# pkzhou/PointSLOT

Hardware: AMD Instinct MI355X
Metric: tracked frames/sec KITTI stereo 1242x375 (higher is better)
Workload: dtype u8

## Files before the change

include/pointslot_hip.h:

```cpp
#ifndef POINTSLOT_HIP_H
#define POINTSLOT_HIP_H

#include <stddef.h>
#include <stdint.h>

#ifdef __cplusplus
extern "C" {
#endif

typedef enum ps_status {
  PS_OK = 0,
  PS_ERR_INVALID = -1,
  PS_ERR_HIP = -2,
  PS_ERR_CAPACITY = -3,
  PS_ERR_NO_DEVICE = -4
} ps_status;

typedef struct ps_keypoint {
  float x, y;
  float size;
  float angle;
  float response;
  int32_t octave;
  int32_t class_id;
} ps_keypoint;

const char* ps_last_error(void);
int ps_device_count(int* count);
const char* ps_version(void);
int ps_debug_poison_lds(int device, uint32_t pattern);
int ps_debug_mfma_f64_peak(int device, double* tflops);
int ps_debug_traffic_kernel(int device, int mode, size_t bytes, int repeats);
void* ps_pinned_alloc(size_t bytes);
void ps_pinned_free(void* p);

typedef struct ps_orb ps_orb;

typedef struct ps_orb_config {
  int32_t nfeatures;
  float scale_factor;
  int32_t nlevels;
  int32_t ini_th_fast;
  int32_t min_th_fast;
  int32_t max_batch;
  int32_t device;
} ps_orb_config;

int ps_orb_create(const ps_orb_config* cfg, ps_orb** out);
void ps_orb_destroy(ps_orb* h);

int ps_orb_get_tables(const ps_orb* h, float* scale_factors, float* inv_scale_factors,
                      float* level_sigma2, float* inv_level_sigma2, int32_t* features_per_level);

int ps_orb_level_size(const ps_orb* h, int w, int hgt, int level, int32_t* w_l, int32_t* h_l);

int ps_orb_extract(ps_orb* h, const uint8_t* img, int w, int hgt, int stride, ps_keypoint* kps,
                   uint8_t* desc, int cap, int* n, uint8_t* const* pyramid_out);

int ps_orb_extract_masked(ps_orb* h, const uint8_t* img, const uint8_t* mask, int w, int hgt, int stride, int mask_stride,
                          ps_keypoint* kps, uint8_t* desc, int cap, int* n);

typedef struct ps_cvorb ps_cvorb;
int ps_cvorb_create(int nfeatures, float scale_factor, int nlevels, int edge_threshold, int fast_threshold, int device, ps_cvorb** out);
void ps_cvorb_destroy(ps_cvorb* h);
int ps_cvorb_detect_and_compute(ps_cvorb* h, const uint8_t* img, const uint8_t* mask, int w, int hgt, int stride, int mask_stride,
                                ps_keypoint* kps, uint8_t* desc, int cap, int* n);
int ps_cvorb_debug_read(ps_cvorb* h, int level, int what, void* out, size_t out_bytes, int* n);

int ps_cvorb_detect_batch_device(ps_cvorb* h, const uint8_t* d_imgs, const uint8_t* d_masks, int nimg, int w, int hgt, int stride,
                                 size_t image_pitch, int mask_stride, size_t mask_pitch, void* stream);
int ps_cvorb_batch_device_outputs(const ps_cvorb* h, const ps_keypoint** d_kps, const uint8_t** d_desc, const int32_t** d_counts,
                                  const int32_t** d_overflow, int32_t* capacity);
int ps_cvorb_batch_fetch(ps_cvorb* h, int image, ps_keypoint* kps, uint8_t* desc, int cap, int* n);

int ps_orb_extract_batch_device(ps_orb* h, const uint8_t* d_imgs, int nimg, int w, int hgt, int stride,
                                size_t image_pitch, void* stream);
int ps_orb_batch_device_outputs(const ps_orb* h, const ps_keypoint** d_kps, const uint8_t** d_desc,
                                const int32_t** d_counts, int32_t* kp_capacity);
int ps_orb_batch_fetch(ps_orb* h, int image, ps_keypoint* kps, uint8_t* desc, int cap, int* n);
int ps_orb_sync(ps_orb* h);

int ps_orb_extract_batch(ps_orb* h, const uint8_t* const* imgs, int nimg, int w, int hgt, int stride);

int ps_orb_stereo_match_batch(ps_orb* h, int npairs, float mb, float mbf);
int ps_orb_stereo_device_outputs(const ps_orb* h, const float** d_uright, const float** d_depth, const int32_t** d_kept);
int ps_orb_stereo_fetch(ps_orb* h, int pair, float* u_right, float* depth, int cap, int* n_left, int* kept);
int ps_orb_stereo_match_pair(ps_orb* left, ps_orb* right, float mb, float mbf, float* u_right, float* depth, int cap, int* n_left);
typedef struct ps_stereo_frame {
  ps_keypoint* kps; uint8_t* desc; float* u_right; float* depth;
  int32_t cap;
  int32_t n, n_right, kept;
} ps_stereo_frame;
int ps_orb_stereo_fetch_frames(ps_orb* h, ps_stereo_frame* frames, int npairs);
int ps_orb_stereo_match_keys(ps_orb* left, ps_orb* right, const ps_keypoint* kps_l, const uint8_t* desc_l, int n_left,
                             const ps_keypoint* kps_r, const uint8_t* desc_r, int n_right, float mb, float mbf,
                             float* u_right, float* depth, int* kept);

int ps_orb_debug_read(ps_orb* h, int image, int level, int what, void* out, size_t out_bytes, int* n);

int ps_orb_stage_times(ps_orb* h, const char** names, float* ms, int cap, int* n);
int ps_orb_enable_stage_timing(ps_orb* h, int enable);

typedef struct ps_matcher ps_matcher;
int ps_matcher_create(int device, ps_matcher** out);
void ps_matcher_destroy(ps_matcher* m);
int ps_matcher_last_kernel_ms(const ps_matcher* m, float* ms);

int ps_hamming_matrix(ps_matcher* m, const uint8_t* q, int nq, const uint8_t* t, int nt, uint16_t* out);

int ps_distinctive_descriptors(ps_matcher* m, const uint8_t* desc, const int32_t* off, int npoints, int32_t* best);

typedef struct ps_bf_problem {
  const uint8_t* q_desc; const float* q_angle; const uint8_t* q_valid; int32_t nq;
  const uint8_t* t_desc; const float* t_angle; int32_t nt;
  int32_t* query_of_train;
// ... 287 lines not shown
```

pointslot_amd/csrc/cvorb_host.hip:

```cpp
#include <hip/hip_runtime.h>
#include <math.h>
#include <stdlib.h>
#include <string.h>
#include <algorithm>
#include <vector>
#include "../../include/pointslot_hip.h"
#include "cvorb_plan.h"
#include "ps_common.h"

extern "C" {
void psk_cv_level0(const CvLevelDev*, const uint8_t*, int, const uint8_t*, int, hipStream_t);
void psk_cv_resize(const CvLevelDev*, const CvLevelDev*, const int4*, const int4*, hipStream_t);
void psk_cv_detect(const CvLevelDev*, int, int, int, int32_t*, hipStream_t);
void psk_cv_blur(const CvLevelDev*, const int*, hipStream_t);
void psk_cv_describe(const CvPlanDev*, const CvSel*, int, void*, uint8_t*, hipStream_t);
void psk_cvb_run(const CvbPlan*, int, const uint8_t*, int, size_t, const uint8_t*, int, size_t, int, hipStream_t);
}

struct ps_cvorb {
  int nfeatures, nlevels, edge, fast_th, device;
  double scale_factor;
  hipStream_t stream = nullptr;
  int w = 0, h = 0;
  bool planned = false;
// ... 289 lines not shown
int ps_cvorb_debug_read(ps_cvorb* h, int level, int what, void* out, size_t out_bytes, int* n) {
  if (!h || !h->planned || level < 0 || level >= h->nlevels || !out) return ps_set_error(PS_ERR_INVALID, "ps_cvorb_debug_read: bad argument");
  PS_HIP(hipSetDevice(h->device));
  if (h->last_fast) {
    const int rc = single_host_selected(h, h->w, h->last_had_mask, nullptr, nullptr, 0, nullptr);
    if (rc != PS_OK) return rc;
  }
  PS_HIP(hipDeviceSynchronize());
  const CvLevelDev& L = h->plan.lv[level];
  if (what == 4) { if (out_bytes < 8) return ps_set_error(PS_ERR_CAPACITY, "buffer too small"); ((int32_t*)out)[0] = L.w; ((int32_t*)out)[1] = L.h; return PS_OK; }
  if (what == 3) {
    const std::vector<float>& c = h->last_cand[level];
    if (c.size() * 4 > out_bytes) return ps_set_error(PS_ERR_CAPACITY, "buffer too small");
    if (!c.empty()) memcpy(out, c.data(), c.size() * 4);
    if (n) *n = (int)(c.size() / 4);
    return PS_OK;
  }
  if ((size_t)L.w * L.h > out_bytes) return ps_set_error(PS_ERR_CAPACITY, "buffer too small");
  if (what == 0) PS_HIP(hipMemcpy2D(out, L.w, L.pad + (size_t)CV_BORDER * L.stride + CV_BORDER, L.stride, L.w, L.h, hipMemcpyDeviceToHost));
  else if (what == 1) PS_HIP(hipMemcpy2D(out, L.w, L.blur + (size_t)CV_BORDER * L.stride + CV_BORDER, L.stride, L.w, L.h, hipMemcpyDeviceToHost));
  else if (what == 2) { if (h->last_had_mask) PS_HIP(hipMemcpy(out, L.mask, (size_t)L.w * L.h, hipMemcpyDeviceToHost)); else memset(out, 0, (size_t)L.w * L.h); }
  else return ps_set_error(PS_ERR_INVALID, "unknown `what` %d", what);
  return PS_OK;
}

}

namespace {
int build_batch_plan(ps_cvorb* h, int w, int hgt, int cap) {
  if (h->b_buf) { hipFree(h->b_buf); h->b_buf = nullptr; }
  h->bplanned = false;
  CvbPlan& P = h->bplan;
  memset(&P, 0, sizeof(P));
  P.nlevels = h->nlevels; P.edge = h->edge; P.fast_th = h->fast_th; P.w0 = w; P.h0 = hgt;
  P.ocw = (w + 7) / 8; P.och = (hgt + 7) / 8;
  if (P.ocw > 512) return ps_set_error(PS_ERR_INVALID, "the batched object detector supports images up to 4096 pixels wide");
  {
    const int hp = 15;
    int v, v0, vmax = cv_floor(hp * sqrtf(2.f) / 2 + 1), vmin = cv_ceil(hp * sqrtf(2.f) / 2);
    for (v = 0; v <= vmax; ++v) P.umax[v] = cv_round(sqrt((double)hp * hp - v * v));
    for (v = hp, v0 = 0; v >= vmin; --v) { while (P.umax[v0] == P.umax[v0 + 1]) ++v0; P.umax[v] = v0; ++v0; }
    static const int disc[16] = {15, 15, 15, 15, 14, 14, 14, 13, 13, 12, 11, 10, 9, 8, 6, 3};
    for (v = 0; v <= hp; ++v)
      if (P.umax[v] != disc[v]) return ps_set_error(PS_ERR_INVALID, "the intensity-centroid disc differs from the kernels' mask table");
  }
  for (int i = 0; i < 4; i++) P.kq[i] = h->kq[i];
  std::vector<int> quota(h->nlevels, 0);
  {
    const float factor = (float)(1.0 / h->scale_factor);
    float ndesired = h->nfeatures * (1 - factor) / (1 - (float)pow((double)factor, (double)h->nlevels));
    int sum = 0;
    for (int l = 0; l < h->nlevels - 1; l++) { quota[l] = cv_round(ndesired); sum += quota[l]; ndesired *= factor; }
    quota[h->nlevels - 1] = std::max(h->nfeatures - sum, 0);
  }
  std::vector<std::vector<int4>> xt(h->nlevels), yt(h->nlevels);
  size_t img_off = 0;
  auto take_img = [&](size_t bytes) { size_t r = img_off; img_off += al(bytes + 64); return r; };
  for (int l = 0; l < h->nlevels; l++) {
    CvbLevel& L = P.lv[l];
    L.scale = (float)pow(h->scale_factor, (double)l);
    const float inv_scale = 1.0f / L.scale;
    L.w = cv_round(w * inv_scale); L.h = cv_round(hgt * inv_scale);
    if (L.w <= 2 * h->edge || L.h <= 2 * h->edge || L.w <= 2 * 24 || L.h <= 2 * 24)
      return ps_set_error(PS_ERR_INVALID, "image %dx%d: level %d is %dx%d, too small for the detector", w, hgt, l, L.w, L.h);
    L.stride = (int)((L.w + 2 * CV_BORDER + 63) / 64 * 64);
    L.tw = (L.w + 2 * CV_BORDER + CVB_TILE - 1) / CVB_TILE; L.th = (L.h + 2 * CV_BORDER + CVB_TILE - 1) / CVB_TILE;
    if (L.tw * L.th > CVB_MAX_TILES) return ps_set_error(PS_ERR_INVALID, "the batched object detector supports levels of up to %d tiles", CVB_MAX_TILES);
    L.cw = (L.w + 2 * CV_BORDER + 7) / 8; L.ch = (L.h + 2 * CV_BORDER + 7) / 8;
    L.cw = std::max(L.cw, 4 * L.tw); L.ch = std::max(L.ch, 4 * L.th);
    L.cw = (L.cw + 3) & ~3;
    if (L.cw > 1024 || L.ch > 512) return ps_set_error(PS_ERR_INVALID, "image too large for the batched object detector's planning kernel");
    L.cell_off = P.cell_total; P.cell_total += L.cw * L.ch; P.cell_max = std::max(P.cell_max, L.cw * L.ch);
    L.tile_off = P.tile_total; P.tile_total += L.tw * L.th;
    L.quota = quota[l];
    L.o_pad = take_img((size_t)L.stride * (L.h + 2 * CV_BORDER)); L.o_blur = take_img((size_t)L.stride * (L.h + 2 * CV_BORDER));
    L.o_mask = take_img((size_t)L.w * L.h); L.o_score = 0;
    if (l > 0) {
      exact_table(P.lv[l - 1].w, L.w, xt[l], &L.sx, &L.dminx, &L.dmaxx); exact_table(P.lv[l - 1].h, L.h, yt[l], &L.sy, &L.dminy, &L.dmaxy);
      if ((double)P.lv[l - 1].w / L.w * 32 + 6 > 48 || (double)P.lv[l - 1].h / L.h * 32 + 6 > 48)
        return ps_set_error(PS_ERR_INVALID, "the batched object detector supports scale factors up to 1.3");
    }
  }
  P.arena_pitch = img_off;
  P.ocap = 2048;
  int max_tiles = 0;
  for (int l = 0; l < h->nlevels; l++) max_tiles = std::max(max_tiles, P.lv[l].tw * P.lv[l].th);
  P.wl_cap = cap * max_tiles;
  if (2 * (size_t)P.cell_total + 2 * (size_t)P.cell_max + 2 * (size_t)(P.ocw + 1) * (P.och + 1) + P.tile_total + 64 > 150 * 1024 || P.tile_total > 8 * 512) return ps_set_error(PS_ERR_INVALID, "image too large for the batched object detector's planning kernel");
  size_t off = 0;
  auto take = [&](size_t bytes) { size_t r = off; off += al(bytes + 64); return r; };
  const size_t o_arena = take(P.arena_pitch * (size_t)cap);
  std::vector<size_t> o_xt(h->nlevels, 0), o_yt(h->nlevels, 0);
  for (int l = 1; l < h->nlevels; l++) { o_xt[l] = take(xt[l].size() * 16); o_yt[l] = take(yt[l].size() * 16); }
  const size_t o_wl = take((size_t)3 * CV_MAX_LEVELS * P.wl_cap * 4);
  const size_t o_kpmap = take((size_t)cap * P.cell_total);
  const size_t o_cand = take((size_t)cap * h->nlevels * CVB_CAND_CAP * sizeof(float4));
  const size_t o_sel = take((size_t)cap * h->nlevels * CVB_CAND_CAP * sizeof(CvSel));
  const size_t o_kps = take((size_t)cap * P.ocap * sizeof(ps_keypoint)), o_desc = take((size_t)cap * P.ocap * 32);
  const size_t o_dump = take(1024);
  const size_t z0 = off;
  const size_t o_occ = take((size_t)cap * P.ocw * P.och), o_wlc = take(3 * CV_MAX_LEVELS * 4), o_ncand = take((size_t)cap * h->nlevels * 4);
  const size_t o_nsel = take((size_t)cap * h->nlevels * 4), o_count = take((size_t)cap * 4), o_ovf = take((size_t)cap * 4);
  const size_t z1 = off;
  hipError_t e = hipMalloc(&h->b_buf, off);
  if (e != hipSuccess) return ps_set_error(PS_ERR_HIP, "hipMalloc(%zu): %s", off, hipGetErrorString(e));
  uint8_t* D = h->b_buf;
  if (const char* fill = getenv("PS_DEBUG_FILL")) PS_HIP(hipMemsetAsync(D, atoi(fill), off, h->stream));
  P.arena = D + o_arena;
  for (int l = 1; l < h->nlevels; l++) {
    P.lv[l].xtab = (const int4*)(D + o_xt[l]); P.lv[l].ytab = (const int4*)(D + o_yt[l]);
    PS_HIP(hipMemcpyAsync(D + o_xt[l], xt[l].data(), xt[l].size() * 16, hipMemcpyHostToDevice, h->stream));
    PS_HIP(hipMemcpyAsync(D + o_yt[l], yt[l].data(), yt[l].size() * 16, hipMemcpyHostToDevice, h->stream));
  }
  P.wl = (uint32_t*)(D + o_wl); P.cand = (float4*)(D + o_cand); P.sel = (CvSel*)(D + o_sel);
  P.kps = (ps_keypoint_pod*)(D + o_kps); P.desc = D + o_desc; P.dump = D + o_dump;
  P.occ = D + o_occ; P.kpmap = D + o_kpmap; P.wl_count = (int32_t*)(D + o_wlc); P.ncand = (int32_t*)(D + o_ncand); P.nsel = (int32_t*)(D + o_nsel);
  P.count = (int32_t*)(D + o_count); P.overflow = (int32_t*)(D + o_ovf);
  h->b_zero = D + z0; h->b_zero_bytes = z1 - z0;
  PS_HIP(hipStreamSynchronize(h->stream));
  h->bw = w; h->bh = hgt; h->bcap = cap; h->bplanned = true;
  return PS_OK;
}
}

extern "C" {
hipStream_t psi_cvorb_stream(ps_cvorb* h) { return h->stream; }

int psi_cvorb_batch_begin(ps_cvorb* h, int nimg, int w, int hgt, hipStream_t st, uint8_t** occ, int* ocw, int* och) {
  if (!h->bplanned || h->bw != w || h->bh != hgt || h->bcap < nimg) {
    int rc = build_batch_plan(h, w, hgt, nimg);
    if (rc != PS_OK) return rc;
  }
  PS_HIP(hipMemsetAsync(h->b_zero, 0, h->b_zero_bytes, st));
  if (occ) *occ = h->bplan.occ;
  if (ocw) *ocw = h->bplan.ocw;
  if (och) *och = h->bplan.och;
  return PS_OK;
}
int psi_cvorb_batch_run(ps_cvorb* h, const uint8_t* d_imgs, const uint8_t* d_masks, int nimg, int stride, size_t image_pitch, int mask_stride,
                        size_t mask_pitch, int occupancy_given, hipStream_t st) {
  psk_cvb_run(&h->bplan, nimg, d_imgs, stride, image_pitch, d_masks, mask_stride, mask_pitch, occupancy_given, st);
  PS_HIP(hipGetLastError());
  h->b_last_n = nimg;
  return PS_OK;
}

int psi_cvorb_batch_worklist_counts(ps_cvorb* h, int32_t* counts , int32_t* tiles ) {
  if (!h || !h->bplanned || !counts || !tiles) return ps_set_error(PS_ERR_INVALID, "no batch plan yet");
  PS_HIP(hipSetDevice(h->device));
  PS_HIP(hipDeviceSynchronize());
  PS_HIP(hipMemcpy(counts, h->bplan.wl_count, 3 * CV_MAX_LEVELS * 4, hipMemcpyDeviceToHost));
  for (int l = 0; l < CV_MAX_LEVELS; l++) tiles[l] = l < h->nlevels ? h->bplan.lv[l].tw * h->bplan.lv[l].th : 0;
  return PS_OK;
}

int ps_cvorb_detect_batch_device(ps_cvorb* h, const uint8_t* d_imgs, const uint8_t* d_masks, int nimg, int w, int hgt, int stride, size_t image_pitch,
                                 int mask_stride, size_t mask_pitch, void* stream) {
  if (!h || !d_imgs || !d_masks || nimg < 1 || w < 1 || hgt < 1 || stride < w || mask_stride < w)
    return ps_set_error(PS_ERR_INVALID, "ps_cvorb_detect_batch_device: bad argument");
  PS_HIP(hipSetDevice(h->device));
  hipStream_t st = stream ? (hipStream_t)stream : h->stream;
  int rc = psi_cvorb_batch_begin(h, nimg, w, hgt, st, nullptr, nullptr, nullptr);
  if (rc != PS_OK) return rc;
  return psi_cvorb_batch_run(h, d_imgs, d_masks, nimg, stride, image_pitch, mask_stride, mask_pitch, 0, st);
}

int ps_cvorb_batch_device_outputs(const ps_cvorb* h, const ps_keypoint** d_kps, const uint8_t** d_desc, const int32_t** d_counts,
                                  const int32_t** d_overflow, int32_t* capacity) {
  if (!h || !h->bplanned) return ps_set_error(PS_ERR_INVALID, "no batch plan yet");
  if (d_kps) *d_kps = (const ps_keypoint*)h->bplan.kps;
  if (d_desc) *d_desc = h->bplan.desc;
  if (d_counts) *d_counts = h->bplan.count;
  if (d_overflow) *d_overflow = h->bplan.overflow;
  if (capacity) *capacity = h->bplan.ocap;
  return PS_OK;
}

int ps_cvorb_batch_fetch(ps_cvorb* h, int image, ps_keypoint* kps, uint8_t* desc, int cap, int* n) {
  if (!h || !h->bplanned || image < 0 || image >= h->b_last_n || !n) return ps_set_error(PS_ERR_INVALID, "ps_cvorb_batch_fetch: bad argument");
  PS_HIP(hipSetDevice(h->device));
  PS_HIP(hipDeviceSynchronize());
  int32_t cnt = 0, ovf = 0;
  PS_HIP(hipMemcpy(&cnt, h->bplan.count + image, 4, hipMemcpyDeviceToHost));
  PS_HIP(hipMemcpy(&ovf, h->bplan.overflow + image, 4, hipMemcpyDeviceToHost));
  if (ovf) return ps_set_error(PS_ERR_CAPACITY, "image %d: more than %d FAST keypoints under the mask on a level, or more than %d keypoints in all", image, CVB_CAND_CAP, h->bplan.ocap);
  *n = cnt;
  if (cnt > cap) return ps_set_error(PS_ERR_CAPACITY, "%d keypoints, caller capacity %d", cnt, cap);
  if (cnt > 0) {
    if (!kps || !desc) return ps_set_error(PS_ERR_INVALID, "null output buffer");
    PS_HIP(hipMemcpy(kps, (const ps_keypoint*)h->bplan.kps + (size_t)image * h->bplan.ocap, (size_t)cnt * sizeof(ps_keypoint), hipMemcpyDeviceToHost));
    PS_HIP(hipMemcpy(desc, h->bplan.desc + (size_t)image * h->bplan.ocap * 32, (size_t)cnt * 32, hipMemcpyDeviceToHost));
  }
  return PS_OK;
}
}
```

pointslot_amd/csrc/cvorb_kernels.hip:

```cpp
#include <hip/hip_runtime.h>
#include <stdint.h>
#include <stdlib.h>
#include "cvorb_plan.h"
#include "retain_best.h"

namespace {

#include "describe_common.h"

__constant__ __attribute__((aligned(16))) int8_t cv_pattern[1024] = {
#include "orb_pattern.inc"
};

__device__ __forceinline__ int reflect101(int p, int len) {
  if (len == 1) return 0;
  while (p < 0 || p >= len) p = p < 0 ? -p : 2 * (len - 1) - p;
  return p;
}

__global__ __launch_bounds__(256) void cv_level0(CvLevelDev L, const uint8_t* img, int stride, const uint8_t* mask, int mask_stride) {
  const int px = blockIdx.x * 256 + threadIdx.x, py = blockIdx.y;
  const int PW = L.w + 2 * CV_BORDER;
  if (px >= PW) return;
  const int x = reflect101(px - CV_BORDER, L.w), y = reflect101(py - CV_BORDER, L.h);
  L.pad[(size_t)py * L.stride + px] = img[(size_t)y * stride + x];
  const int ix = px - CV_BORDER, iy = py - CV_BORDER;
  if (L.mask && ix >= 0 && ix < L.w && iy >= 0 && iy < L.h) L.mask[(size_t)iy * L.w + ix] = mask[(size_t)iy * mask_stride + ix];
}

__device__ __forceinline__ uint32_t cv_hline(const uint8_t* S, int sw, int4 tx) {
  if (tx.w == 1) return (uint32_t)S[0] << 8;
  if (tx.w == 2) return (uint32_t)S[sw - 1] << 8;
  return (uint32_t)tx.y * S[tx.x] + (uint32_t)tx.z * S[tx.x + 1];
}
__device__ __forceinline__ uint8_t cv_interp(const uint8_t* src, int sstride, int sw, int sh, int4 tx, int4 ty) {
  if (ty.w != 0) {
    const uint32_t v = cv_hline(src + (size_t)(ty.w == 1 ? 0 : sh - 1) * sstride, sw, tx);
    return (uint8_t)min((v + 128u) >> 8, 255u);
  }
  const uint32_t r0 = cv_hline(src + (size_t)ty.x * sstride, sw, tx), r1 = cv_hline(src + (size_t)(ty.x + 1) * sstride, sw, tx);
  const unsigned long long v = (unsigned long long)r0 * (uint32_t)ty.y + (unsigned long long)r1 * (uint32_t)ty.z;
  return (uint8_t)min((v + 32768ull) >> 16, 255ull);
}
__global__ __launch_bounds__(256) void cv_resize(CvLevelDev L, CvLevelDev P, const int4* xtab, const int4* ytab) {
  const int px = blockIdx.x * 256 + threadIdx.x, py = blockIdx.y;
  const int PW = L.w + 2 * CV_BORDER;
  if (px >= PW) return;
  const int x = reflect101(px - CV_BORDER, L.w), y = reflect101(py - CV_BORDER, L.h);
  const int4 tx = xtab[x], ty = ytab[y];
  const uint8_t* proi = P.pad + (size_t)CV_BORDER * P.stride + CV_BORDER;
  L.pad[(size_t)py * L.stride + px] = cv_interp(proi, P.stride, P.w, P.h, tx, ty);
  const int ix = px - CV_BORDER, iy = py - CV_BORDER;
  if (L.mask && ix >= 0 && ix < L.w && iy >= 0 && iy < L.h) {
    const uint8_t m = cv_interp(P.mask, P.w, P.w, P.h, tx, ty);
    L.mask[(size_t)iy * L.w + ix] = m > 254 ? m : 0;
  }
}

__global__ __launch_bounds__(256) void cv_score(CvLevelDev L, int th) {
  const int x = blockIdx.x * 256 + threadIdx.x, y = blockIdx.y;
  if (x >= L.w) return;
  uint8_t out = 0;
  if (x >= 3 && x < L.w - 3 && y >= 3 && y < L.h - 3) {
    const uint8_t* c = L.pad + (size_t)(CV_BORDER + y) * L.stride + CV_BORDER + x;
    const int st = L.stride, v = c[0];
    const int n = c[3 * st], e = c[3], so = c[-3 * st], w = c[-3];
    const int M = min(min(max(n, e), max(e, so)), min(max(so, w), max(w, n)));
    const int m = max(max(min(n, e), min(e, so)), max(min(so, w), min(w, n)));
    if (v - M > th || m - v > th) {
      const int off[16] = {3 * st, 3 * st + 1, 2 * st + 2, st + 3, 3, -st + 3, -2 * st + 2, -3 * st + 1,
                           -3 * st, -3 * st - 1, -2 * st - 2, -st - 3, -3, st - 3, 2 * st - 2, 3 * st - 1};
      int r[16];
#pragma unroll
      for (int i = 0; i < 16; i++) r[i] = c[off[i]];
      int best = 0;
#pragma unroll
      for (int k = 0; k < 16; k++) {
        int mx = r[k], mn = r[k];
#pragma unroll
        for (int j = 1; j < 9; j++) { mx = max(mx, r[(k + j) & 15]); mn = min(mn, r[(k + j) & 15]); }
        best = max(best, max(v - mx, mn - v));
      }
      if (best > th) out = (uint8_t)best;
    }
  }
  L.score[(size_t)y * L.w + x] = out;
}
// ... 103 lines not shown
__global__ __launch_bounds__(64) void cv_describe(CvPlanDev plan, const CvSel* sel, int nsel, ps_keypoint_pod* kps, uint8_t* desc) {
  const int k = blockIdx.x, lane = threadIdx.x;
  if (k >= nsel) return;
  const CvSel S = sel[k];
  const CvLevelDev& L = plan.lv[S.level];
  const int x0 = S.x, y0 = S.y;
  const uint8_t* center = L.pad + (size_t)(CV_BORDER + y0) * L.stride + CV_BORDER + x0;
  int m10 = 0, m01 = 0;
  if (lane <= 15) {
    const int v = lane, d = plan.umax[v];
    if (v == 0) {
      for (int u = -15; u <= 15; ++u) m10 += u * center[u];
    } else {
      int v_sum = 0;
      for (int u = -d; u <= d; ++u) {
        const int vp = center[u + v * L.stride], vm = center[u - v * L.stride];
        v_sum += vp - vm;
        m10 += u * (vp + vm);
      }
      m01 = v * v_sum;
    }
  }
#pragma unroll
  for (int dd = 32; dd >= 1; dd >>= 1) { m10 += __shfl_xor(m10, dd); m01 += __shfl_xor(m01, dd); }
  const float angle_deg = cv_fast_atan2_deg((float)m01, (float)m10);
  const float px = __fmul_rn((float)x0, L.scale), py = __fmul_rn((float)y0, L.scale);
  if (lane == 0) {
    ps_keypoint_pod o;
    o.x = px; o.y = py; o.size = __fmul_rn(31.f, L.scale); o.angle = angle_deg; o.response = S.response; o.octave = S.level; o.class_id = -1;
    kps[k] = o;
  }
  if (lane < 32) {
    const float inv = __fdiv_rn(1.f, L.scale);
    const float angle = __fmul_rn(angle_deg, (float)(3.14159265358979323846 / 180.f));
    const float a = (float)cos((double)angle), b = (float)sin((double)angle);
    const uint8_t* c = L.blur + (size_t)(CV_BORDER + __float2int_rn(__fmul_rn(py, inv))) * L.stride + CV_BORDER + __float2int_rn(__fmul_rn(px, inv));
    const int8_t* pat = cv_pattern + lane * 32;
    int val = 0;
    for (int t = 0; t < 8; t++) {
      int tv[2];
      for (int q = 0; q < 2; q++) {
        const float fx = (float)pat[4 * t + 2 * q], fy = (float)pat[4 * t + 2 * q + 1];
        const float rx = __fsub_rn(__fmul_rn(fx, a), __fmul_rn(fy, b)), ry = __fadd_rn(__fmul_rn(fx, b), __fmul_rn(fy, a));
        tv[q] = c[__float2int_rn(ry) * L.stride + __float2int_rn(rx)];
      }
      val |= (tv[0] < tv[1]) << t;
    }
    desc[(size_t)k * 32 + lane] = (uint8_t)val;
  }
}


__device__ __forceinline__ CvLevelDev cvb_level(const CvbPlan& P, int img, int l) {
  const CvbLevel& B = P.lv[l];
  uint8_t* base = P.arena + (size_t)img * P.arena_pitch;
  CvLevelDev L;
  L.w = B.w; L.h = B.h; L.stride = B.stride; L.scale = B.scale;
  L.pad = base + B.o_pad; L.blur = base + B.o_blur; L.mask = base + B.o_mask; L.score = nullptr;
  L.rowcnt = nullptr; L.rowoff = nullptr; L.cand = nullptr;
  return L;
}

__global__ __launch_bounds__(256) void cvb_occupancy(CvbPlan P, const uint8_t* masks, int mask_stride, size_t mask_pitch) {
  __shared__ uint8_t flag[4][512];
  const int img = blockIdx.y, band = blockIdx.x, tid = threadIdx.x;
  for (int i = tid; i < 4 * 512; i += 256) (&flag[0][0])[i] = 0;
  __syncthreads();
  const uint8_t* M = masks + (size_t)img * mask_pitch;
  for (int x = tid; x < P.w0; x += 256)
    for (int b = 0; b < 4; b++) {
      const int y0 = band * 32 + b * 8, y1 = min(y0 + 8, P.h0);
      uint32_t any = 0;
      for (int y = y0; y < y1; y++) any |= M[(size_t)y * mask_stride + x];
      if (any) flag[b][x >> 3] = 1;
    }
  __syncthreads();
  uint8_t* occ = P.occ + (size_t)img * P.ocw * P.och;
  for (int i = tid; i < 4 * P.ocw; i += 256) {
    const int b = i / P.ocw, cx = i % P.ocw, cy = band * 4 + b;
    if (cy < P.och) occ[cy * P.ocw + cx] = flag[b][cx];
  }
}

__device__ __forceinline__ void cvb_reflect_range(int lo, int hi, int len, int& rlo, int& rhi) {
  rlo = 1 << 30; rhi = -1;
  if (lo < 0) { const int a = -min(hi, 0), b = -lo; rlo = min(rlo, a); rhi = max(rhi, b); }
  if (hi >= 0 && lo <= len - 1) { rlo = min(rlo, max(lo, 0)); rhi = max(rhi, min(hi, len - 1)); }
  if (hi > len - 1) { const int a = 2 * (len - 1) - hi, b = 2 * (len - 1) - max(lo, len - 1); rlo = min(rlo, a); rhi = max(rhi, b); }
  rlo = max(rlo, 0); rhi = min(rhi, len - 1);
}

#ifndef CVB_PLAN_T
#define CVB_PLAN_T 512
#endif
#define CVB_PLAN_MAXCW 1024
#define CVB_PLAN_MAXCH 512
#ifdef PS_CVP_PROFILE
#define CPP_DECL long long cp_t = wall_clock64(), cp_ph[8] = {0, 0, 0, 0, 0, 0, 0, 0}
#define CPP_MARK(k) do { const long long _n = wall_clock64(); cp_ph[k] += _n - cp_t; cp_t = _n; } while (0)
#define CPP_PRINT() do { if (threadIdx.x == 0 && blockIdx.x == 0) printf("cvb_plan ticks: sat %lld | cells %lld fast+rowdil %lld coldil %lld blurtiles %lld | down %lld wl0 %lld entries %lld\n", cp_ph[0], cp_ph[1], cp_ph[2], cp_ph[3], cp_ph[4], cp_ph[5], cp_ph[6], cp_ph[7]); } while (0)
#else
#define CPP_DECL
#define CPP_MARK(k)
#define CPP_PRINT()
#endif
__global__ __launch_bounds__(CVB_PLAN_T) void cvb_plan(CvbPlan P) {
  extern __shared__ uint8_t sm[];
  const int img = blockIdx.x, tid = threadIdx.x, lane = tid & 63, wave = tid >> 6, NW = CVB_PLAN_T / 64;
  CPP_DECL;
  const int cmax4 = (P.cell_max + 3) & ~3;
  uint8_t* kp = sm + ((P.cell_total + 3) & ~3);
  uint8_t* tmp = kp + cmax4;
  uint16_t* sat = reinterpret_cast<uint16_t*>(tmp + cmax4);
  uint8_t* tflag = reinterpret_cast<uint8_t*>(sat + (P.ocw + 1) * (P.och + 1));
  __shared__ int s_cnt[3 * CV_MAX_LEVELS], s_base[3 * CV_MAX_LEVELS];
  __shared__ uint32_t s_xr[CVB_PLAN_MAXCW];
  __shared__ uint8_t s_kprow[CVB_PLAN_MAXCH], s_drow[CVB_PLAN_MAXCH];
  for (int i = tid; i < P.tile_total; i += CVB_PLAN_T) tflag[i] = 0;
  if (tid < 3 * CV_MAX_LEVELS) s_cnt[tid] = 0;
  const uint8_t* occ = P.occ + (size_t)img * P.ocw * P.och;
  uint8_t* kpmap = P.kpmap + (size_t)img * P.cell_total;
  const int SW = P.ocw + 1;
  for (int y = wave; y <= P.och; y += NW)
    for (int x = lane; x < SW; x += 64) sat[y * SW + x] = (y > 0 && x > 0) ? occ[(y - 1) * P.ocw + x - 1] : 0;
  __syncthreads();
  for (int y = 1 + tid; y <= P.och; y += CVB_PLAN_T) { uint16_t acc = 0; for (int x = 1; x <= P.ocw; x++) { acc += sat[y * SW + x]; sat[y * SW + x] = acc; } }
  __syncthreads();
  for (int x = 1 + tid; x <= P.ocw; x += CVB_PLAN_T) { uint16_t acc = 0; for (int y = 1; y <= P.och; y++) { acc += sat[y * SW + x]; sat[y * SW + x] = acc; } }
  __syncthreads();
  CPP_MARK(0);
  for (int l = 0; l < P.nlevels; l++) {
    const CvbLevel& B = P.lv[l];
    uint8_t* need = sm + B.cell_off;
    const int cw4 = B.cw >> 2;
    uint32_t* need4 = reinterpret_cast<uint32_t*>(need);
    uint32_t* kp4 = reinterpret_cast<uint32_t*>(kp);
    uint32_t* tmp4 = reinterpret_cast<uint32_t*>(tmp);
    uint32_t* kpmap4 = reinterpret_cast<uint32_t*>(kpmap + B.cell_off);
    const float Rx = (float)P.w0 / (float)B.w, Ry = (float)P.h0 / (float)B.h;
    const float mx = 6.f * (Rx - 1.f) + 3.f, my = 6.f * (Ry - 1.f) + 3.f;
    for (int cx = tid; cx < B.cw; cx += CVB_PLAN_T) {
      const int x0 = max(8 * cx - CV_BORDER, 0), x1 = min(8 * cx - CV_BORDER + 7, B.w - 1);
      uint32_t e = 0xFFFFFFFFu;
      if (x0 <= x1) {
        const int X0 = max((int)floorf((float)x0 * Rx - mx), 0) >> 3, X1 = min((int)ceilf((float)(x1 + 1) * Rx + mx), P.w0 - 1) >> 3;
        e = (uint32_t)X0 | ((uint32_t)X1 << 16);
      }
      s_xr[cx] = e;
    }
    __syncthreads();
    for (int cy = wave; cy < B.ch; cy += NW) {
      const int y0 = max(8 * cy - CV_BORDER, 0), y1 = min(8 * cy - CV_BORDER + 7, B.h - 1);
      bool anyrow = false;
      int Y0 = 0, Y1 = 0, band = 0;
      if (y0 <= y1) {
        Y0 = max((int)floorf((float)y0 * Ry - my), 0) >> 3; Y1 = min((int)ceilf((float)(y1 + 1) * Ry + my), P.h0 - 1) >> 3;
        band = (int)sat[(Y1 + 1) * SW + P.ocw] - (int)sat[Y0 * SW + P.ocw];
      }
      if (band > 0) {
        for (int cx = lane; cx < B.cw; cx += 64) {
          const uint32_t e = s_xr[cx];
          bool any = false;
          if (e != 0xFFFFFFFFu) {
            const int X0 = (int)(e & 0xFFFFu), X1 = (int)(e >> 16);
            const int cnt = (int)sat[(Y1 + 1) * SW + X1 + 1] - (int)sat[Y0 * SW + X1 + 1] - (int)sat[(Y1 + 1) * SW + X0] + (int)sat[Y0 * SW + X0];
            any = cnt > 0;
          }
          const int c = cy * B.cw + cx;
          kp[c] = any ? 1 : 0;
          need[c] = any ? 2 : 0;
          kpmap[B.cell_off + c] = any ? 1 : 0;
          anyrow = anyrow || any;
        }
        anyrow = __any(anyrow);
      } else {
        for (int q = lane; q < cw4; q += 64) { kp4[cy * cw4 + q] = 0; need4[cy * cw4 + q] = 0; kpmap4[cy * cw4 + q] = 0; }
      }
      if (lane == 0) s_kprow[cy] = anyrow ? 1 : 0;
    }
    __syncthreads();
    CPP_MARK(1);
    for (int ty = wave; ty < B.th; ty += NW) {
      bool rows = false;
      for (int cy = max(4 * ty - 1, 0); cy <= min(4 * ty + 4, B.ch - 1); cy++) rows = rows || s_kprow[cy];
      if (!rows) continue;
      for (int tx = lane; tx < B.tw; tx += 64) {
        uint32_t acc = 0;
        for (int cy = max(4 * ty - 1, 0); cy <= min(4 * ty + 4, B.ch - 1); cy++) {
          const uint32_t cur = kp4[cy * cw4 + tx];
          const uint32_t prv = tx > 0 ? kp4[cy * cw4 + tx - 1] & 0xFF000000u : 0u, nxt = tx + 1 < cw4 ? kp4[cy * cw4 + tx + 1] & 0xFFu : 0u;
          acc |= cur | prv | nxt;
        }
        if (acc) tflag[B.tile_off + ty * B.tw + tx] |= 2u;
      }
    }
    for (int cy = wave; cy < B.ch; cy += NW) {
      if (!s_kprow[cy]) { for (int q = lane; q < cw4; q += 64) tmp4[cy * cw4 + q] = 0; continue; }
      for (int q = lane; q < cw4; q += 64) {
        const uint32_t cur = kp4[cy * cw4 + q], prv = q > 0 ? kp4[cy * cw4 + q - 1] : 0u, nxt = q + 1 < cw4 ? kp4[cy * cw4 + q + 1] : 0u;
        uint32_t v = cur;
        v |= __builtin_amdgcn_alignbyte(cur, prv, 1u) | __builtin_amdgcn_alignbyte(cur, prv, 2u) | __builtin_amdgcn_alignbyte(cur, prv, 3u);
        v |= __builtin_amdgcn_alignbyte(nxt, cur, 1u) | __builtin_amdgcn_alignbyte(nxt, cur, 2u) | __builtin_amdgcn_alignbyte(nxt, cur, 3u);
        tmp4[cy * cw4 + q] = v;
      }
    }
    __syncthreads();
    CPP_MARK(2);
    for (int cy = wave; cy < B.ch; cy += NW) {
      bool rows = false;
      for (int y = max(cy - 3, 0); y <= min(cy + 3, B.ch - 1); y++) rows = rows || s_kprow[y];
      if (lane == 0) s_drow[cy] = rows ? 1 : 0;
      if (!rows) { for (int q = lane; q < cw4; q += 64) kp4[cy * cw4 + q] = 0; continue; }
      for (int q = lane; q < cw4; q += 64) {
        uint32_t v = 0;
        for (int y = max(cy - 3, 0); y <= min(cy + 3, B.ch - 1); y++) v |= tmp4[y * cw4 + q];
        kp4[cy * cw4 + q] = v;
        need4[cy * cw4 + q] |= v;
      }
    }
    __syncthreads();
    CPP_MARK(3);
    for (int ty = wave; ty < B.th; ty += NW) {
      bool rows = false;
      for (int cy = 4 * ty; cy <= min(4 * ty + 3, B.ch - 1); cy++) rows = rows || s_drow[cy];
      if (!rows) continue;
      for (int tx = lane; tx < B.tw; tx += 64) {
        uint32_t acc = 0;
        for (int cy = 4 * ty; cy <= min(4 * ty + 3, B.ch - 1); cy++) acc |= kp4[cy * cw4 + tx];
        if (acc) tflag[B.tile_off + ty * B.tw + tx] |= (l == 0 ? 5u : 4u);
      }
    }
    __syncthreads();
  }
  CPP_MARK(4);
  for (int l = P.nlevels - 1; l >= 2; l--) {
    const CvbLevel& B = P.lv[l];
    const CvbLevel& S = P.lv[l - 1];
    uint32_t* down = reinterpret_cast<uint32_t*>(sm + S.cell_off);
    const float rx = (float)S.w / (float)B.w, ry = (float)S.h / (float)B.h;
    for (int cy = wave; cy < B.ch; cy += NW) {
      int ly0, ly1;
      cvb_reflect_range(8 * cy - CV_BORDER, min(8 * cy - CV_BORDER + 7, B.h + CV_BORDER - 1), B.h, ly0, ly1);
      const int sy0 = max((int)floorf(((float)ly0 + 0.5f) * ry - 0.5f) - 1, 0), sy1 = min((int)floorf(((float)ly1 + 0.5f) * ry - 0.5f) + 2, S.h - 1);
      const int ay0 = (sy0 + CV_BORDER) >> 3, ay1 = (sy1 + CV_BORDER) >> 3;
      for (int cx = lane; cx < B.cw; cx += 64) {
        const uint32_t bits = sm[B.cell_off + cy * B.cw + cx];
        if (!bits) continue;
        int lx0, lx1;
        cvb_reflect_range(8 * cx - CV_BORDER, min(8 * cx - CV_BORDER + 7, B.w + CV_BORDER - 1), B.w, lx0, lx1);
        const int sx0 = max((int)floorf(((float)lx0 + 0.5f) * rx - 0.5f) - 1, 0), sx1 = min((int)floorf(((float)lx1 + 0.5f) * rx - 0.5f) + 2, S.w - 1);
        const int ax0 = (sx0 + CV_BORDER) >> 3, ax1 = (sx1 + CV_BORDER) >> 3;
        for (int ay = ay0; ay <= ay1; ay++)
          for (int ax = ax0; ax <= ax1; ax++) {
            const int i = ay * S.cw + ax;
            atomicOr(&down[i >> 2], bits << (8 * (i & 3)));
          }
      }
    }
    __syncthreads();
  }
  CPP_MARK(5);
  for (int l = 1; l < P.nlevels; l++) {
    const CvbLevel& B = P.lv[l];
    const uint8_t* need = sm + B.cell_off;
    for (int ty = wave; ty < B.th; ty += NW)
      for (int tx = lane; tx < B.tw; tx += 64) {
        uint32_t acc = 0;
        for (int cy = 4 * ty; cy < 4 * ty + 4; cy++) acc |= *reinterpret_cast<const uint32_t*>(need + cy * B.cw + 4 * tx);
        uint8_t f = 0;
        if (acc & 0x03030303u) f |= 1;
        if (acc & 0x02020202u) f |= 8;
        tflag[B.tile_off + ty * B.tw + tx] |= f;
      }
  }
  __syncthreads();
  CPP_MARK(6);
  constexpr int PER = 8 * 512 / CVB_PLAN_T;
  int lpos[PER][3];
  for (int k = 0; k < PER; k++) {
    const int i = tid + k * CVB_PLAN_T;
    lpos[k][0] = lpos[k][1] = lpos[k][2] = -1;
    if (i >= P.tile_total) continue;
    int l = 0;
    for (int q = 1; q < P.nlevels; q++) if (i >= P.lv[q].tile_off) l = q;
    const uint8_t f = tflag[i];
    for (int w = 0; w < 3; w++) if ((f >> w) & 1) lpos[k][w] = atomicAdd(&s_cnt[w * CV_MAX_LEVELS + l], 1);
  }
  __syncthreads();
  if (tid < 3 * CV_MAX_LEVELS) s_base[tid] = s_cnt[tid] > 0 ? atomicAdd(&P.wl_count[tid], s_cnt[tid]) : 0;
  __syncthreads();
  for (int k = 0; k < PER; k++) {
    const int i = tid + k * CVB_PLAN_T;
    if (i >= P.tile_total) continue;
    int l = 0;
    for (int q = 1; q < P.nlevels; q++) if (i >= P.lv[q].tile_off) l = q;
    const uint8_t f = tflag[i];
    for (int w = 0; w < 3; w++)
      if (lpos[k][w] >= 0) {
        const int pos = s_base[w * CV_MAX_LEVELS + l] + lpos[k][w];
        if (pos < P.wl_cap) P.wl[((size_t)w * CV_MAX_LEVELS + l) * P.wl_cap + pos] = ((uint32_t)img << 12) | (uint32_t)(i - P.lv[l].tile_off) | ((w == 0 && (f & 8)) ? 0x80000000u : 0u);
      }
  }
  CPP_MARK(7);
  CPP_PRINT();
}

typedef const uint32_t __attribute__((address_space(4))) * cvb_scalar_ptr;
__device__ __forceinline__ uint32_t cvb_sload(const uint32_t* p) { return *(cvb_scalar_ptr)(uintptr_t)p; }
#ifndef CVB_RUN
#define CVB_RUN 1
#endif
#define CVB_TILE_VARS(P, which, l)                                                                      \
  const CvbLevel& B = P.lv[l];                                                                          \
  const uint32_t* wl = P.wl + ((size_t)(which) * CV_MAX_LEVELS + (l)) * P.wl_cap;                       \
  const int cnt = min((int)cvb_sload(reinterpret_cast<const uint32_t*>(P.wl_count) + (which) * CV_MAX_LEVELS + (l)), P.wl_cap); \
  const int xchunk = (cnt + 7) >> 3, xend = min(cnt, ((int)(blockIdx.x & 7) + 1) * xchunk);             \
  const int xstep = (int)(gridDim.x >> 3) * CVB_RUN;                                                    \
  int it = (int)(blockIdx.x & 7) * xchunk + (int)(blockIdx.x >> 3) * CVB_RUN, run_i = 0;                \
  auto cvb_next = [&](int i, int r) { return r + 1 < CVB_RUN ? i + 1 : i + xstep - (CVB_RUN - 1); };    \
  uint32_t e_next = it < xend ? cvb_sload(wl + it) : 0u;
#define CVB_TILE_FOR                                                                                    \
  for (uint32_t e = e_next; it < xend && ((e = e_next), (e_next = cvb_next(it, run_i) < xend ? cvb_sload(wl + cvb_next(it, run_i)) : 0u), true); \
       it = cvb_next(it, run_i), run_i = run_i + 1 < CVB_RUN ? run_i + 1 : 0)
#define CVB_HAS_NEXT (cvb_next(it, run_i) < xend)
#define CVB_TILE_LOOP(P, which, l) CVB_TILE_VARS(P, which, l) CVB_TILE_FOR

#define CVB_TT 64
typedef unsigned short cvb_us2 __attribute__((ext_vector_type(2)));
typedef short cvb_s2 __attribute__((ext_vector_type(2)));
static_assert(CVB_TT == 64, "cvb_wave_sync orders LDS traffic inside ONE wave: the tile kernels must be launched with 64-thread workgroups");
__device__ __forceinline__ void cvb_wave_sync() {
  __builtin_amdgcn_fence(__ATOMIC_RELEASE, "wavefront");
  __builtin_amdgcn_wave_barrier();
  __builtin_amdgcn_fence(__ATOMIC_ACQUIRE, "wavefront");
}
__device__ __forceinline__ int4 cvb_tab_entry(int val, double scale, int ssize, int dmin, int dmax) {
  if (val < dmin) return make_int4(0, 256, 0, 1);
  if (val >= dmax) return make_int4(ssize - 1, 256, 0, 2);
  const double fval = __dsub_rn(__dmul_rn(scale, __dadd_rn((double)val, 0.5)), 0.5);
  const int ival = (int)floor(fval);
  const int c1 = __double2int_rn(__dmul_rn(__dsub_rn(fval, (double)ival), 256.0));
  return make_int4(ival, 256 - c1, c1, 0);
}

__global__ __launch_bounds__(CVB_TT) void cvb_level0(CvbPlan P) {
  const int tid = threadIdx.x;
  CVB_TILE_LOOP(P, 0, 0) {
    const int img = (int)((e >> 12) & 0x7FFFFu), t = (int)(e & 4095u), tx = t % B.tw, ty = t / B.tw;
    const CvLevelDev L = cvb_level(P, img, 0);
    const uint8_t* I = P.imgs + (size_t)img * P.img_pitch;
    const int px0 = CVB_TILE * tx + (tid & 7) * 4;
    int xs[4];
    for (int j = 0; j < 4; j++) xs[j] = reflect101(min(px0 + j, L.w + 2 * CV_BORDER - 1) - CV_BORDER, L.w);
    uint32_t v[4];
// ... 797 lines not shown
```

Measured before the change: 52280.

## Precompute cell down-chain tables and mark all lower levels in one pass

Replaces the per-level sequential downward propagation of need-bits, which ran one level after another with a barrier between each, with precomputed per-cell source-range chain tables in shared memory. Each coarse-level cell then ORs its bits directly into every finer level in a single barrier-free pass. It skips ranges already covered by left and upper neighbours to cut redundant LDS atomics. The chain tables add shared memory and upfront compute. The bit encoding also changes, with propagated bits shifted into higher bit positions and tile flag masks widened to match, so correctness depends on the exact double-precision range math matching the resize.

```diff
diff --git a/include/pointslot_hip.h b/include/pointslot_hip.h
--- a/include/pointslot_hip.h
+++ b/include/pointslot_hip.h
@@ -31,6 +31,8 @@
 int ps_debug_poison_lds(int device, uint32_t pattern);
 int ps_debug_mfma_f64_peak(int device, double* tflops);
 int ps_debug_traffic_kernel(int device, int mode, size_t bytes, int repeats);
+struct ps_cvorb;
+int ps_debug_cvorb_worklist_counts(struct ps_cvorb* h, int32_t* counts, int32_t* tiles);
 void* ps_pinned_alloc(size_t bytes);
 void ps_pinned_free(void* p);
 
diff --git a/pointslot_amd/csrc/cvb_need.h b/pointslot_amd/csrc/cvb_need.h
--- /dev/null
+++ b/pointslot_amd/csrc/cvb_need.h
@@ -0,0 +1,60 @@
+#pragma once
+#include <math.h>
+#include <stdint.h>
+
+#ifdef __HIPCC__
+#define CVN_HD __host__ __device__ __forceinline__
+#else
+#define CVN_HD inline
+#endif
+
+#define CVN_BORDER 23
+
+struct CvnStep { int32_t dlen, slen, dmin, dmax; double scale; };
+
+CVN_HD int cvn_min(int a, int b) { return a < b ? a : b; }
+CVN_HD int cvn_max(int a, int b) { return a > b ? a : b; }
+
+CVN_HD void cvn_reflect_range(int lo, int hi, int len, int& rlo, int& rhi) {
+  rlo = 1 << 30; rhi = -1;
+  if (lo < 0) { const int a = -cvn_min(hi, 0), b = -lo; rlo = cvn_min(rlo, a); rhi = cvn_max(rhi, b); }
+  if (hi >= 0 && lo <= len - 1) { rlo = cvn_min(rlo, cvn_max(lo, 0)); rhi = cvn_max(rhi, cvn_min(hi, len - 1)); }
+  if (hi > len - 1) { const int a = 2 * (len - 1) - hi, b = 2 * (len - 1) - cvn_max(lo, len - 1); rlo = cvn_min(rlo, a); rhi = cvn_max(rhi, b); }
+  rlo = cvn_max(rlo, 0); rhi = cvn_min(rhi, len - 1);
+}
+
+CVN_HD int cvn_ival(int val, double scale) {
+#ifdef __HIP_DEVICE_COMPILE__
+  const double fval = __dsub_rn(__dmul_rn(scale, __dadd_rn((double)val, 0.5)), 0.5);
+#else
+  const double fval = scale * ((double)val + 0.5) - 0.5;
+#endif
+  return (int)floor(fval);
+}
+
+CVN_HD void cvn_src_range(const CvnStep& S, int d0, int d1, int& s0, int& s1) {
+  s0 = d0 < S.dmin ? 0 : (d0 >= S.dmax ? S.slen - 1 : cvn_ival(d0, S.scale));
+  s1 = d1 < S.dmin ? 0 : (d1 >= S.dmax ? S.slen - 1 : cvn_min(cvn_ival(d1, S.scale) + 1, S.slen - 1));
+}
+
+CVN_HD void cvn_cell_chain(const CvnStep* step, int l, int c, uint32_t* out, int stride) {
+  const int lo = 8 * c - CVN_BORDER, hi = cvn_min(lo + 7, step[l].dlen + CVN_BORDER - 1);
+  if (lo > hi) { for (int m = l - 1; m >= 1; m--) out[(m - 1) * stride] = 1u; return; }
+  int d0, d1;
+  cvn_reflect_range(lo, hi, step[l].dlen, d0, d1);
+  for (int m = l - 1; m >= 1; m--) {
+    int s0, s1;
+    cvn_src_range(step[m + 1], d0, d1, s0, s1);
+    out[(m - 1) * stride] = (uint32_t)((s0 + CVN_BORDER) >> 3) | ((uint32_t)((s1 + CVN_BORDER) >> 3) << 16);
+    d0 = s0; d1 = s1;
+  }
+}
+
+CVN_HD bool cvn_occ_range(int c, int len, int len0, int& o0, int& o1) {
+  const int p0 = cvn_max(8 * c - CVN_BORDER, 0), p1 = cvn_min(8 * c - CVN_BORDER + 7, len - 1);
+  if (p0 > p1) return false;
+  const float R = (float)len0 / (float)len, m = 6.f * (R - 1.f) + 3.f;
+  o0 = cvn_max((int)floorf((float)p0 * R - m), 0) >> 3;
+  o1 = cvn_min((int)ceilf((float)(p1 + 1) * R + m), len0 - 1) >> 3;
+  return true;
+}
diff --git a/pointslot_amd/csrc/cvorb_host.hip b/pointslot_amd/csrc/cvorb_host.hip
--- a/pointslot_amd/csrc/cvorb_host.hip
+++ b/pointslot_amd/csrc/cvorb_host.hip
@@ -395,6 +395,11 @@
     }
   }
   P.arena_pitch = img_off;
+  {
+    size_t chain = 0;
+    for (int l = 2; l < h->nlevels; l++) chain += (size_t)4 * (l - 1) * (P.lv[l].cw + P.lv[l].ch);
+    P.cell_max = std::max(P.cell_max, (int)((chain + 1) / 2));
+  }
   P.ocap = 2048;
   int max_tiles = 0;
   for (int l = 0; l < h->nlevels; l++) max_tiles = std::max(max_tiles, P.lv[l].tw * P.lv[l].th);
@@ -466,6 +471,10 @@
   for (int l = 0; l < CV_MAX_LEVELS; l++) tiles[l] = l < h->nlevels ? h->bplan.lv[l].tw * h->bplan.lv[l].th : 0;
   return PS_OK;
 }
+int ps_debug_cvorb_worklist_counts(ps_cvorb* h, int32_t* counts , int32_t* tiles ) {
+  int32_t t[CV_MAX_LEVELS];
+  return psi_cvorb_batch_worklist_counts(h, counts, tiles ? tiles : t);
+}
 
 int ps_cvorb_detect_batch_device(ps_cvorb* h, const uint8_t* d_imgs, const uint8_t* d_masks, int nimg, int w, int hgt, int stride, size_t image_pitch,
                                  int mask_stride, size_t mask_pitch, void* stream) {
diff --git a/pointslot_amd/csrc/cvorb_kernels.hip b/pointslot_amd/csrc/cvorb_kernels.hip
--- a/pointslot_amd/csrc/cvorb_kernels.hip
+++ b/pointslot_amd/csrc/cvorb_kernels.hip
@@ -3,6 +3,7 @@
 #include <stdlib.h>
 #include "cvorb_plan.h"
 #include "retain_best.h"
+#include "cvb_need.h"
 
 namespace {
 
@@ -272,23 +273,16 @@
   }
 }
 
-__device__ __forceinline__ void cvb_reflect_range(int lo, int hi, int len, int& rlo, int& rhi) {
-  rlo = 1 << 30; rhi = -1;
-  if (lo < 0) { const int a = -min(hi, 0), b = -lo; rlo = min(rlo, a); rhi = max(rhi, b); }
-  if (hi >= 0 && lo <= len - 1) { rlo = min(rlo, max(lo, 0)); rhi = max(rhi, min(hi, len - 1)); }
-  if (hi > len - 1) { const int a = 2 * (len - 1) - hi, b = 2 * (len - 1) - max(lo, len - 1); rlo = min(rlo, a); rhi = max(rhi, b); }
-  rlo = max(rlo, 0); rhi = min(rhi, len - 1);
-}
-
 #ifndef CVB_PLAN_T
 #define CVB_PLAN_T 512
 #endif
 #define CVB_PLAN_MAXCW 1024
 #define CVB_PLAN_MAXCH 512
+static_assert(CVN_BORDER == CV_BORDER, "cvb_need.h restates the padded planes' border");
 #ifdef PS_CVP_PROFILE
 #define CPP_DECL long long cp_t = wall_clock64(), cp_ph[8] = {0, 0, 0, 0, 0, 0, 0, 0}
 #define CPP_MARK(k) do { const long long _n = wall_clock64(); cp_ph[k] += _n - cp_t; cp_t = _n; } while (0)
-#define CPP_PRINT() do { if (threadIdx.x == 0 && blockIdx.x == 0) printf("cvb_plan ticks: sat %lld | cells %lld fast+rowdil %lld coldil %lld blurtiles %lld | down %lld wl0 %lld entries %lld\n", cp_ph[0], cp_ph[1], cp_ph[2], cp_ph[3], cp_ph[4], cp_ph[5], cp_ph[6], cp_ph[7]); } while (0)
+#define CPP_PRINT() do { if (threadIdx.x == 0 && blockIdx.x == 0) printf("cvb_plan ticks: sat %lld | cells %lld fast+rowdil %lld coldil %lld blurtiles + chain tables %lld | down marks %lld wl0 %lld entries %lld\n", cp_ph[0], cp_ph[1], cp_ph[2], cp_ph[3], cp_ph[4], cp_ph[5], cp_ph[6], cp_ph[7]); } while (0)
 #else
 #define CPP_DECL
 #define CPP_MARK(k)
@@ -306,6 +300,27 @@
   __shared__ int s_cnt[3 * CV_MAX_LEVELS], s_base[3 * CV_MAX_LEVELS];
   __shared__ uint32_t s_xr[CVB_PLAN_MAXCW];
   __shared__ uint8_t s_kprow[CVB_PLAN_MAXCH], s_drow[CVB_PLAN_MAXCH];
+  __shared__ CvnStep s_step[2][CV_MAX_LEVELS];
+  __shared__ int4 s_lv[CV_MAX_LEVELS + 1], s_lv2[CV_MAX_LEVELS];
+  if (tid == 0) {
+    int item = 0, entry = 0;
+    for (int l = 0; l <= CV_MAX_LEVELS; l++) {
+      const bool on = l >= 2 && l < P.nlevels;
+      s_lv[l] = make_int4(on ? P.lv[l].cw : 0, item, entry, on ? P.lv[l].ch : 0);
+      if (on) { item += P.lv[l].cw + P.lv[l].ch; entry += (l - 1) * (P.lv[l].cw + P.lv[l].ch); }
+    }
+  }
+  if (tid >= 32 && tid < 32 + CV_MAX_LEVELS) { const int l = tid - 32; s_lv2[l] = l < P.nlevels ? make_int4(P.lv[l].cw, P.lv[l].ch, P.lv[l].cell_off, 0) : make_int4(0, 0, 0, 0); }
+  if (tid >= 64 && tid < 64 + 2 * CV_MAX_LEVELS) {
+    const int a = (tid - 64) / CV_MAX_LEVELS, l = (tid - 64) % CV_MAX_LEVELS;
+    CvnStep st = {0, 0, 0, 0, 1.0};
+    if (l >= 1 && l < P.nlevels) {
+      const CvbLevel& B = P.lv[l];
+      const CvbLevel& S = P.lv[l - 1];
+      st.dlen = a ? B.h : B.w; st.slen = a ? S.h : S.w; st.dmin = a ? B.dminy : B.dminx; st.dmax = a ? B.dmaxy : B.dmaxx; st.scale = a ? B.sy : B.sx;
+    }
+    s_step[a][l] = st;
+  }
   for (int i = tid; i < P.tile_total; i += CVB_PLAN_T) tflag[i] = 0;
   if (tid < 3 * CV_MAX_LEVELS) s_cnt[tid] = 0;
   const uint8_t* occ = P.occ + (size_t)img * P.ocw * P.och;
@@ -327,24 +342,15 @@
     uint32_t* kp4 = reinterpret_cast<uint32_t*>(kp);
     uint32_t* tmp4 = reinterpret_cast<uint32_t*>(tmp);
     uint32_t* kpmap4 = reinterpret_cast<uint32_t*>(kpmap + B.cell_off);
-    const float Rx = (float)P.w0 / (float)B.w, Ry = (float)P.h0 / (float)B.h;
-    const float mx = 6.f * (Rx - 1.f) + 3.f, my = 6.f * (Ry - 1.f) + 3.f;
     for (int cx = tid; cx < B.cw; cx += CVB_PLAN_T) {
-      const int x0 = max(8 * cx - CV_BORDER, 0), x1 = min(8 * cx - CV_BORDER + 7, B.w - 1);
-      uint32_t e = 0xFFFFFFFFu;
-      if (x0 <= x1) {
-        const int X0 = max((int)floorf((float)x0 * Rx - mx), 0) >> 3, X1 = min((int)ceilf((float)(x1 + 1) * Rx + mx), P.w0 - 1) >> 3;
-        e = (uint32_t)X0 | ((uint32_t)X1 << 16);
-      }
-      s_xr[cx] = e;
+      int X0, X1;
+      s_xr[cx] = cvn_occ_range(cx, B.w, P.w0, X0, X1) ? (uint32_t)X0 | ((uint32_t)X1 << 16) : 0xFFFFFFFFu;
     }
     __syncthreads();
     for (int cy = wave; cy < B.ch; cy += NW) {
-      const int y0 = max(8 * cy - CV_BORDER, 0), y1 = min(8 * cy - CV_BORDER + 7, B.h - 1);
       bool anyrow = false;
       int Y0 = 0, Y1 = 0, band = 0;
-      if (y0 <= y1) {
-        Y0 = max((int)floorf((float)y0 * Ry - my), 0) >> 3; Y1 = min((int)ceilf((float)(y1 + 1) * Ry + my), P.h0 - 1) >> 3;
+      if (cvn_occ_range(cy, B.h, P.h0, Y0, Y1)) {
         band = (int)sat[(Y1 + 1) * SW + P.ocw] - (int)sat[Y0 * SW + P.ocw];
       }
       if (band > 0) {
@@ -423,32 +429,65 @@
     __syncthreads();
   }
   CPP_MARK(4);
-  for (int l = P.nlevels - 1; l >= 2; l--) {
-    const CvbLevel& B = P.lv[l];
-    const CvbLevel& S = P.lv[l - 1];
-    uint32_t* down = reinterpret_cast<uint32_t*>(sm + S.cell_off);
-    const float rx = (float)S.w / (float)B.w, ry = (float)S.h / (float)B.h;
-    for (int cy = wave; cy < B.ch; cy += NW) {
-      int ly0, ly1;
-      cvb_reflect_range(8 * cy - CV_BORDER, min(8 * cy - CV_BORDER + 7, B.h + CV_BORDER - 1), B.h, ly0, ly1);
-      const int sy0 = max((int)floorf(((float)ly0 + 0.5f) * ry - 0.5f) - 1, 0), sy1 = min((int)floorf(((float)ly1 + 0.5f) * ry - 0.5f) + 2, S.h - 1);
-      const int ay0 = (sy0 + CV_BORDER) >> 3, ay1 = (sy1 + CV_BORDER) >> 3;
-      for (int cx = lane; cx < B.cw; cx += 64) {
-        const uint32_t bits = sm[B.cell_off + cy * B.cw + cx];
-        if (!bits) continue;
-        int lx0, lx1;
-        cvb_reflect_range(8 * cx - CV_BORDER, min(8 * cx - CV_BORDER + 7, B.w + CV_BORDER - 1), B.w, lx0, lx1);
-        const int sx0 = max((int)floorf(((float)lx0 + 0.5f) * rx - 0.5f) - 1, 0), sx1 = min((int)floorf(((float)lx1 + 0.5f) * rx - 0.5f) + 2, S.w - 1);
-        const int ax0 = (sx0 + CV_BORDER) >> 3, ax1 = (sx1 + CV_BORDER) >> 3;
-        for (int ay = ay0; ay <= ay1; ay++)
-          for (int ax = ax0; ax <= ax1; ax++) {
-            const int i = ay * S.cw + ax;
-            atomicOr(&down[i >> 2], bits << (8 * (i & 3)));
+  uint32_t* chain = reinterpret_cast<uint32_t*>(kp);
+  for (int i = tid; i < s_lv[P.nlevels].y; i += CVB_PLAN_T) {
+    int l = 2;
+    while (l + 1 < P.nlevels && i >= s_lv[l + 1].y) l++;
+    const int4 v = s_lv[l];
+    const int c = i - v.y;
+    if (c < v.x) cvn_cell_chain(s_step[0], l, c, chain + v.z + c, v.x);
+    else cvn_cell_chain(s_step[1], l, c - v.x, chain + v.z + (l - 1) * v.x + (c - v.x), v.w);
+  }
+  __syncthreads();
+  CPP_MARK(4);
+  {
+    int first = wave;
+    for (int l = 2; l < P.nlevels; l++) {
+      const CvbLevel& B = P.lv[l];
+      const uint32_t* tabx = chain + s_lv[l].z;
+      const uint32_t* taby = tabx + (l - 1) * B.cw;
+      int cy = first;
+      for (; cy < B.ch; cy += NW) {
+        const int cw4 = B.cw >> 2;
+        const uint32_t* own4 = reinterpret_cast<const uint32_t*>(sm + B.cell_off) + cy * cw4;
+        bool any = false;
+        for (int q = lane; q < cw4; q += 64) any = any || (own4[q] & 0x03030303u) != 0u;
+        if (!__any(any)) continue;
+        for (int it = lane; it < cw4 * (l - 1); it += 64) {
+          const int q = it % cw4, m = 1 + it / cw4;
+          const uint32_t cur = own4[q] & 0x03030303u;
+          if (!cur) continue;
+          const uint32_t up = cy > 0 ? own4[q - cw4] & 0x03030303u : 0u;
+          const uint32_t left = q > 0 ? (own4[q - 1] >> 24) & 3u : 0u;
+          const int4 S = s_lv2[m];
+          uint32_t* down = reinterpret_cast<uint32_t*>(sm + S.z);
+          const uint32_t* tx = tabx + (m - 1) * B.cw + 4 * q;
+          const uint32_t yr = taby[(m - 1) * B.ch + cy], yu = cy > 0 ? taby[(m - 1) * B.ch + cy - 1] : 1u;
+          uint32_t xn = q > 0 ? tx[-1] : 1u;
+          const int ay1 = min((int)(yr >> 16), S.y - 1);
+#pragma unroll
+          for (int j = 0; j < 4; j++) {
+            const uint32_t bits = (cur >> (8 * j)) & 3u, xr = tx[j];
+            const uint32_t lb = j > 0 ? (cur >> (8 * (j - 1))) & 3u : left, ub = (up >> (8 * j)) & 3u;
+            const uint32_t xl = xn;
+            xn = xr;
+            if (!bits) continue;
+            int ax0 = (int)(xr & 0xFFFFu), ay0 = (int)(yr & 0xFFFFu);
+            const int ax1 = min((int)(xr >> 16), S.x - 1);
+            if ((lb & bits) == bits && (int)(xl & 0xFFFFu) <= ax0) ax0 = max(ax0, (int)(xl >> 16) + 1);
+            if ((ub & bits) == bits && (int)(yu & 0xFFFFu) <= ay0) ay0 = max(ay0, (int)(yu >> 16) + 1);
+            for (int ay = ay0; ay <= ay1; ay++)
+              for (int ax = ax0; ax <= ax1; ax++) {
+                const int i = ay * S.x + ax;
+                atomicOr(&down[i >> 2], (bits << 2) << (8 * (i & 3)));
+              }
           }
-      }
-    }
-    __syncthreads();
-  }
+        }
+      }
+      first = cy - B.ch;
+    }
+  }
+  __syncthreads();
   CPP_MARK(5);
   for (int l = 1; l < P.nlevels; l++) {
     const CvbLevel& B = P.lv[l];
@@ -458,8 +497,8 @@
         uint32_t acc = 0;
         for (int cy = 4 * ty; cy < 4 * ty + 4; cy++) acc |= *reinterpret_cast<const uint32_t*>(need + cy * B.cw + 4 * tx);
         uint8_t f = 0;
-        if (acc & 0x03030303u) f |= 1;
-        if (acc & 0x02020202u) f |= 8;
+        if (acc & 0x0F0F0F0Fu) f |= 1;
+        if (acc & 0x0A0A0A0Au) f |= 8;
         tflag[B.tile_off + ty * B.tw + tx] |= f;
       }
   }
```

Measured after the change: 52930 (median of 6 runs). 1.01x the previous value.
